# SiftScience/kafka-assigner

Hardware: AMD Instinct MI355X
Metric: assignment scenarios/sec at 100k partitions x 1k brokers RF=3 (higher is better)
Workload: dtype int32

## Files before the change

kafka-assigner_amd/csrc/kas_first_fit.h:

```cpp
#pragma once

namespace kas {

#ifndef KAS_P4_U
#define KAS_P4_U 4
#endif
#ifndef KAS_P4_U_WIDE
#define KAS_P4_U_WIDE 1
#endif
template <int W, int NW, int NC = NW>
KAS_DEV void p4_lists_parallel(const LdsView& L, const TopicView& T, int32_t live_count, int32_t wave,
                               int64_t (&st)[8], int32_t& fail_win, int32_t& fail_row, uint64_t* fin = nullptr, uint64_t fin_hi = 0ull) {
  const int lane = kasw::lane();
  uint64_t* prog = (uint64_t*)&L.ctl[KAS_CTL_PROG];
  int32_t oc[NC], total = 0;
#pragma unroll
  for (int w = 0; w < NC; ++w) { oc[w] = L.ctl[KAS_CTL_OC + w]; total += oc[w]; }
  auto orphan_row = [&](int32_t g) -> int32_t {
    int32_t w = 0, base = 0;
#pragma unroll
    for (int k = 0; k < NC - 1; ++k) {
      const bool next = w == k && g >= base + oc[k];
      base += next ? oc[k] : 0;
      w += next ? 1 : 0;
    }
    return g < total ? T.orph[((int64_t)chunk_begin<NC>(T.nt, w) << 6) + (g - base)] : -1;
  };
  auto row_cells = [&](int32_t p) -> MidRaw<W> {
    return mid_load_raw<W>(T.mid, T.ow, p >= 0 ? p : 0, p >= 0, T.m32);
  };
  const int32_t n_win = (total + 63) >> 6;
  const int32_t dw = (lane >= 1 && lane < NW) ? lane : 1;
  const int32_t xw = (wave + NW - dw) % NW;
  const int32_t cap = T.cap, mw = mid_width(T.ow);
  constexpr int U = W >= 4 ? KAS_P4_U_WIDE : KAS_P4_U;
  int32_t p_nxt = orphan_row(64 * wave + lane);
  MidRaw<W> c_nxt = row_cells(p_nxt);
  for (int32_t w = wave; w < n_win; w += NW) {
    const int32_t p = p_nxt;
    int32_t c_cur[W];
    mid_unpack<W>(c_nxt, T.ow, c_cur, T.m32);
    p_nxt = orphan_row(64 * (w + NW) + lane);
    c_nxt = row_cells(p_nxt);
    kasw::repoll();
    if (kasw::ballot(L.ctl[KAS_CTL_FAILWIN] < w) != 0) break;
    int32_t hc = 0, hr[W];
#pragma unroll
    for (int k = 0; k < W; ++k) {
      hr[k] = (p >= 0 && c_cur[k] >= 0) ? (int32_t)lds_rack(L, c_cur[k]) : -1;
      hc += (p >= 0 && c_cur[k] >= 0) ? 1 : 0;
    }
    int32_t need = p >= 0 ? T.rf - hc : 0;
    int32_t j = kasw::shfl(L.ctl[KAS_CTL_HEAD], 0);
    if (lane == 0) prog[wave] = ((uint64_t)(uint32_t)w << 32) | (uint32_t)j;
    KAS_COUNT(st[4]);
    bool stop = false;
    bool placed = false;
    for (;;) {
      uint64_t pend = kasw::ballot(need > 0);
      if (pend == 0) break;
      if (j >= live_count) {
        if (lane == 0) kasw::lds_atomic_min(&L.ctl[KAS_CTL_FAILWIN], w);
        stop = true;
        break;
      }
      int32_t n[U], slots[U], rk[U];
#pragma unroll
      for (int u = 0; u < U; ++u) n[u] = (int32_t)L.live[j + u < live_count ? j + u : j];
#pragma unroll
      for (int u = 0; u < U; ++u) rk[u] = (int32_t)lds_rack(L, n[u]);
      if (w > 0 && NW > 1) {
        const int32_t upto = j + U < live_count ? j + U : live_count;
        const bool watch = lane >= 1 && lane < NW && w - dw >= 0;
        const uint64_t want = ((uint64_t)(uint32_t)(w - dw) << 32) + (uint32_t)upto;
        bool abandoned = false;
        int32_t idle = 0;
        for (;;) {
          kasw::repoll();
          if (kasw::ballot(watch && prog[xw] < want) == 0) break;
          if (kasw::ballot(L.ctl[KAS_CTL_FAILWIN] < w) != 0) { abandoned = true; break; }
          if (watchdog_poll((uint32_t*)&L.ctl[KAS_CTL_WATCHDOG], false, idle)) {
            if (lane == 0) kasw::lds_atomic_min(&L.ctl[KAS_CTL_FAILWIN], -1);
            abandoned = true;
            break;
          }
        }
        if (abandoned) { stop = true; break; }
      }
#pragma unroll
      for (int u = 0; u < U; ++u) slots[u] = cap - lds_load(L, n[u]);
      int32_t taken[U];
#pragma unroll
      for (int u = 0; u < U; ++u) {
        taken[u] = 0;
        if (j + u < live_count && pend != 0) {
          KAS_COUNT(st[5]);
          if (slots[u] > 0) {
            bool want = need > 0;
#pragma unroll
            for (int k = 0; k < W; ++k) want = want && !(k < hc && hr[k] == rk[u]);
            const uint64_t wm = kasw::ballot(want);
            if (wm != 0) {
              const int32_t rank = kasw::count_below(wm);
              if (want && rank < slots[u]) {
                if (W == 3 && T.m32) {
                  put<W>(c_cur, hc, n[u]);
                  placed = true;
                } else {
                  T.mid[(int64_t)p * mw + hc] = (uint16_t)n[u];
                }
                put<W>(hr, hc, rk[u]);
                hc += 1;
                need -= 1;
              }
              const int32_t takers = kasw::popc(wm);
              taken[u] = takers < slots[u] ? takers : slots[u];
              pend = kasw::ballot(need > 0);
            }
          }
        }
      }
      if (lane == 0) {
#pragma unroll
        for (int u = 0; u < U; ++u) if (taken[u] > 0) lds_load(L, n[u]) = cap - slots[u] + taken[u];
      }
      kasw::lockstep();
      j += U;
      if (lane == 0) prog[wave] = ((uint64_t)(uint32_t)w << 32) | (uint32_t)(j < live_count ? j : live_count);
    }
    if constexpr (W == 3) {
      if (T.m32 && placed) reinterpret_cast<uint32_t*>(T.mid)[p] = mid32_pack(c_cur[0], c_cur[1], c_cur[2]);
    }
    if (stop) {
      if (j >= live_count) {
        const uint64_t left = kasw::ballot(need > 0);
        fail_win = w;
        fail_row = kasw::shfl(p, left != 0 ? kasw::first_lane(left) : 0);
      }
      if (lane == 0) prog[wave] = (uint64_t)(uint32_t)(w + 1) << 32;
      break;
    }
    if (lane == 0) {
      int32_t head = L.ctl[KAS_CTL_HEAD];
      while (head < live_count && lds_load(L, (int32_t)L.live[head]) >= cap) ++head;
      kasw::lds_atomic_max(&L.ctl[KAS_CTL_HEAD], head);
      prog[wave] = (uint64_t)(uint32_t)(w + 1) << 32;
    }
    if (fin != nullptr) {
      const int32_t nxt0 = kasw::shfl(p_nxt, 0);
      kasw::wave_sync();
      if (lane == 0) kasw::store_shared_u64_lds(fin, fin_hi | (uint64_t)(uint32_t)(nxt0 >= 0 ? nxt0 : T.P));
    }
  }
}

KAS_DEV void first_fit_reset_ctl(const LdsView& L, int32_t tid) {
  if (tid < KAS_CTL_INTS) L.ctl[tid] = tid == KAS_CTL_FAILROW ? -1 : (tid == KAS_CTL_FAILWIN ? 0x7fffffff : 0);
}

KAS_DEV int32_t first_fit_live_list(const LdsView& L, const TopicView& T, int32_t idxN) {
  const int lane = kasw::lane();
  const int32_t N = T.N, cap = T.cap;
  const int32_t start = (N - idxN) % N;
  int32_t live_count = 0;
  for (int32_t base = 0; base < N; base += 64) {
    const int32_t j = base + lane;
    int32_t n = j + start; if (n >= N) n -= N;
    const bool is_live = j < N && lds_load(L, n) < cap;
    const uint64_t m = kasw::ballot(is_live);
    if (is_live) L.live[live_count + kasw::count_below(m)] = (int16_t)n;
    live_count += kasw::popc(m);
  }
  kasw::lockstep();
  if (lane == 0) L.ctl[KAS_CTL_LIVE] = live_count;
  return live_count;
}

KAS_DEV bool first_fit_hung(const LdsView& L) { return KAS_SPIN_BOUND > 0 && L.ctl[KAS_CTL_WATCHDOG] != 0; }

KAS_DEV TopicOutcome first_fit_outcome(const LdsView& L, const TopicView& T, bool hung) {
  TopicOutcome o;
  o.status = KAS_OK; o.fail_partition = -1; o.moved_replicas = 0; o.moved_partitions = 0;
  const int32_t row = hung ? -1 : L.ctl[KAS_CTL_FAILROW];
  if (hung) o.status = KAS_FAIL_WATCHDOG;
  else if (row >= 0) {
    o.status = KAS_FAIL_UNASSIGNABLE;
    o.fail_partition = T.pid_arr ? T.pid_arr[row] : row;
  }
  return o;
}

template <int W, int NW, int NC = NW, bool FS = false>
KAS_DEV void first_fit_windows(const LdsView& L, const TopicView& T, int32_t wave, int64_t (&st)[8], uint64_t* fin = nullptr, uint64_t fin_hi = 0ull) {
  const int lane = kasw::lane();
  if constexpr (FS) {
    int32_t total_o = 0;
#pragma unroll
    for (int w = 0; w < NC; ++w) total_o += L.ctl[KAS_CTL_OC + w];
    int32_t first = T.P;
    if (total_o > 0) {
      int32_t w0 = 0;
      while (w0 < NC - 1 && L.ctl[KAS_CTL_OC + w0] == 0) ++w0;
      first = T.orph[(int64_t)chunk_begin<NC>(T.nt, w0) << 6];
    }
    if (lane == 0) kasw::store_shared_u64_lds(fin, fin_hi | (uint64_t)(uint32_t)first);
  }
  int32_t fail_win = -1, fail_row = -1;
  p4_lists_parallel<W, NW, NC>(L, T, L.ctl[KAS_CTL_LIVE], wave, st, fail_win, fail_row, fin, fin_hi);
  if constexpr (FS) kasw::wave_sync(); else kasw::sync();
  if (fail_win >= 0 && fail_win == L.ctl[KAS_CTL_FAILWIN] && lane == 0) L.ctl[KAS_CTL_FAILROW] = fail_row;
}

template <int W, int NW, int NC = NW, bool FS = false>
KAS_DEV TopicOutcome first_fit_topic(const LdsView& L, const TopicView& T, int64_t (&st)[8], uint64_t* fin = nullptr, uint64_t fin_hi = 0ull) {
  static_assert(!FS || NW == 1, "first fit inside the order kernel's workgroup is one wavefront");
  const int32_t wave = FS ? 0 : kasw::wave_id();
  auto barrier = [&]() { if constexpr (FS) kasw::wave_sync(); else kasw::sync(); };
  if (wave == 0) first_fit_live_list(L, T, java_abs_mod(T.hash, T.N));
  barrier();
  first_fit_windows<W, NW, NC, FS>(L, T, wave, st, fin, fin_hi);
  barrier();
  return first_fit_outcome(L, T, first_fit_hung(L));
}

template <int W, int PW, bool FS = false, int M32C = -1>
KAS_DEV void p4_scenario(const KasLaunch& a, int32_t s, unsigned char* lds_raw, uint64_t* fs = nullptr) {
  constexpr int NW = PW, NT = 64 * NW, NC = KAS_P4_WAVES;
  const int lane = kasw::lane();
  const int tid = FS ? lane : kasw::tid();
  auto barrier = [&]() { if constexpr (FS) kasw::wave_sync(); else kasw::sync(); };
  const kas_scenario_desc sd = a.scen[s];
  const int32_t N = sd.n_nodes;
  const KasP4Lds lay = kas_p4_lds_layout(a.n_max);
  LdsView L;
  L.x = nullptr; L.qrs = nullptr; L.idmap = nullptr; L.ids = nullptr; L.ring_p = nullptr; L.ring_meta = nullptr; L.ring_rack = nullptr;
  L.load = (int32_t*)(lds_raw + lay.off_load);
  L.rack = (int16_t*)(lds_raw + lay.off_rack);
  L.live = (int16_t*)(lds_raw + lay.off_live);
  L.ctl = (int32_t*)(lds_raw + lay.off_ctl);
  L.ns = 1; L.rs = 1;
  const int32_t* g_node_rack = a.node_rack + sd.node_off;
  const int64_t t_begin = kasw::clock_ticks();
  int64_t st[8] = {0, 0, 0, 0, 0, 0, 0, 0};
  int32_t* orph = a.orph + a.orph_off[s];
  bool failed = false;
  int32_t moved_r = 0, moved_p = 0;
  for (int32_t k = 0; k < sd.topic_count; ++k) {
    const int32_t ti = sd.topic_begin + k;
    const kas_topic_desc td = a.topics[ti];
    int32_t* const orph_topic = orph;
    orph += (int64_t)((td.n_partitions > 0 ? td.n_partitions : 0) + 63) / 64 * 64;
    if (failed) {
      out_pad(topic_out(a, td), (int64_t)td.n_partitions * td.out_width, tid, NT);
      TopicOutcome o;
      o.status = KAS_SKIPPED; o.fail_partition = -1; o.moved_replicas = 0; o.moved_partitions = 0;
      if (tid == 0) put_topic_result(a, ti, o);
      continue;
    }
    const kas_topic_result tr0 = a.topic_results[ti];
    moved_r += tr0.moved_replicas; moved_p += tr0.moved_partitions;
    const int32_t* p4s = a.p4s + (int64_t)ti * (KAS_P4S_HEAD + a.n_max);
    if (tr0.status != KAS_OK || p4s[0] == 0) {
      if constexpr (FS) {
        if (lane == 0) kasw::store_shared_u64_lds(&fs[0], ((uint64_t)(uint32_t)k << 32) | (uint64_t)(uint32_t)(td.n_partitions > 0 ? td.n_partitions : 0));
      }
      continue;
    }
    TopicView T = topic_view(a, td, N, M32C);
    T.orph = orph_topic;
    T.cap = p4s[1];
    barrier();
    for (int32_t i = tid; i < N; i += NT) { L.load[i] = p4s[KAS_P4S_HEAD + i]; L.rack[i] = (int16_t)g_node_rack[i]; }
    first_fit_reset_ctl(L, tid);
    barrier();
    if (tid < NC) L.ctl[KAS_CTL_OC + tid] = p4s[2 + tid];
    TopicOutcome o = first_fit_topic<W, NW, NC, FS>(L, T, st, FS ? &fs[0] : nullptr, (uint64_t)(uint32_t)k << 32);
    if (o.status != KAS_OK) {
      failed = true;
      moved_r -= tr0.moved_replicas; moved_p -= tr0.moved_partitions;
      if constexpr (FS) {
        if (lane == 0) kasw::store_shared_u64_lds(&fs[1], (uint64_t)(uint32_t)k);
        int32_t idle = 0;
        for (;;) {
          kasw::repoll();
          if (kasw::ballot(kasw::load_shared_u64_lds(&fs[2]) != 0ull) != 0ull) break;
          if (watchdog_poll(reinterpret_cast<uint32_t*>(&fs[3]), false, idle)) break;
        }
      }
      out_pad(topic_out(a, td), (int64_t)td.n_partitions * td.out_width, tid, NT);
      if (tid == 0) {
        put_topic_result(a, ti, o);
        put_scenario_result(a, s, o.status, k, o.fail_partition, moved_r, moved_p);
      }
    }
  }
  if constexpr (FS) {
    kasw::wave_sync();
    if (lane == 0) kasw::store_shared_u64_lds(&fs[0], (uint64_t)(uint32_t)sd.topic_count << 32);
  }
  if (tid == 0 && a.stats) a.stats[(int64_t)s * KAS_STATS_PER_SCENARIO + 3] += kasw::clock_ticks() - t_begin;
}

}
```

Before: 678,000.

## Prefetch orphan lists two windows ahead with async inline-asm global loads

Replaces the per-row orphan-index search with precomputed prefix/step offsets, and issues orphan-list and mid-row loads as asynchronous inline-asm global loads two windows ahead. Waiting is deferred until after the placement loop, so memory latency overlaps with the first-fit work. The new path is used only for single-wave forms with a compile-time M32C. It adds hand-written asm with s_nop and explicit waits, plus template specialisations for full-width rows.

```diff
diff --git a/kafka-assigner_amd/csrc/kas_first_fit.h b/kafka-assigner_amd/csrc/kas_first_fit.h
--- a/kafka-assigner_amd/csrc/kas_first_fit.h
+++ b/kafka-assigner_amd/csrc/kas_first_fit.h
@@ -8,42 +8,123 @@
 #ifndef KAS_P4_U_WIDE
 #define KAS_P4_U_WIDE 1
 #endif
-template <int W, int NW, int NC = NW>
+KAS_DEV void first_fit_request_u32(uint32_t& dst, const void* base, uint32_t voff) {
+#if defined(__HIP_DEVICE_COMPILE__)
+  asm volatile("s_nop 4\n\tglobal_load_dword %0, %1, %2 offset:0" : "+v"(dst) : "v"(voff), "s"(base) : "memory");
+#else
+  kasw::gload_u32_async<0>(dst, base, voff);
+#endif
+}
+KAS_DEV void first_fit_request_u16(uint32_t& dst, const void* base, uint32_t voff) {
+#if defined(__HIP_DEVICE_COMPILE__)
+  asm volatile("s_nop 4\n\tglobal_load_ushort %0, %1, %2 offset:0" : "+v"(dst) : "v"(voff), "s"(base) : "memory");
+#else
+  kasw::gload_u16_async<0>(dst, base, voff);
+#endif
+}
+template <int W, bool M32, bool FULLW>
+KAS_DEV void first_fit_rows_request(MidRaw<W>& r, const uint16_t* mid, int32_t ow, int32_t p) {
+  if constexpr (M32) {
+    first_fit_request_u32(r.w[0], mid, (uint32_t)p * 4u);
+  } else if constexpr (FULLW) {
+    const uint32_t off = (uint32_t)p * (uint32_t)(2 * mid_width_of<W>());
+#pragma unroll
+    for (int k = 0; k < W / 2; ++k) first_fit_request_u32(r.w[k], mid, off + 4u * (uint32_t)k);
+    if constexpr (W & 1) first_fit_request_u16(r.w[W / 2], mid, off + 2u * (uint32_t)(W - 1));
+  } else {
+    const uint32_t off = (uint32_t)p * (uint32_t)(2 * mid_width(ow));
+#pragma unroll
+    for (int k = 0; k < W; ++k) first_fit_request_u16(r.w[k], mid, off + 2u * (uint32_t)(k < ow ? k : ow - 1));
+  }
+}
+template <int W, bool M32, bool FULLW>
+KAS_DEV MidRaw<W> first_fit_rows_take(const MidRaw<W>& r, int32_t ow, bool active) {
+  MidRaw<W> o;
+#pragma unroll
+  for (int k = 0; k < W; ++k) o.w[k] = 0xffffffffu;
+  if constexpr (M32) {
+    if (active) o.w[0] = r.w[0];
+  } else if constexpr (FULLW) {
+#pragma unroll
+    for (int k = 0; k < W / 2; ++k) if (active) o.w[k] = r.w[k];
+    if constexpr (W & 1) if (active) o.w[W / 2] = r.w[W / 2] | 0xffff0000u;
+  } else {
+#pragma unroll
+    for (int k = 0; k < W; ++k) if (active && k < ow) o.w[k] = r.w[k];
+  }
+  return o;
+}
+
+template <int W, int NW, int NC = NW, int AS = -1, bool FULLW = false>
 KAS_DEV void p4_lists_parallel(const LdsView& L, const TopicView& T, int32_t live_count, int32_t wave,
                                int64_t (&st)[8], int32_t& fail_win, int32_t& fail_row, uint64_t* fin = nullptr, uint64_t fin_hi = 0ull) {
+  static_assert(AS < 0 || NW == 1, "the asynchronous requests are the one-wavefront forms'");
+  static_assert(AS != 1 || W == 3, "dword mid rows: lists 3 wide");
   const int lane = kasw::lane();
   uint64_t* prog = (uint64_t*)&L.ctl[KAS_CTL_PROG];
-  int32_t oc[NC], total = 0;
-#pragma unroll
-  for (int w = 0; w < NC; ++w) { oc[w] = L.ctl[KAS_CTL_OC + w]; total += oc[w]; }
-  auto orphan_row = [&](int32_t g) -> int32_t {
-    int32_t w = 0, base = 0;
-#pragma unroll
-    for (int k = 0; k < NC - 1; ++k) {
-      const bool next = w == k && g >= base + oc[k];
-      base += next ? oc[k] : 0;
-      w += next ? 1 : 0;
-    }
-    return g < total ? T.orph[((int64_t)chunk_begin<NC>(T.nt, w) << 6) + (g - base)] : -1;
-  };
-  auto row_cells = [&](int32_t p) -> MidRaw<W> {
-    return mid_load_raw<W>(T.mid, T.ow, p >= 0 ? p : 0, p >= 0, T.m32);
-  };
+  int32_t pre[NC], step[NC], total = 0;
+#pragma unroll
+  for (int k = 0; k < NC; ++k) {
+    pre[k] = total;
+    step[k] = (chunk_begin<NC>(T.nt, k) << 6) - (k > 0 ? (chunk_begin<NC>(T.nt, k - 1) << 6) + kasw::uniform(L.ctl[KAS_CTL_OC + k - 1]) : 0);
+    total += kasw::uniform(L.ctl[KAS_CTL_OC + k]);
+  }
   const int32_t n_win = (total + 63) >> 6;
+  if (wave >= n_win) return;
+  auto orphan_entry = [&](int32_t g) -> uint32_t {
+    int32_t e = g + step[0];
+#pragma unroll
+    for (int k = 1; k < NC; ++k) e += g >= pre[k] ? step[k] : 0;
+    return g < total ? (uint32_t)e : 0u;
+  };
+  const int32_t* const uorph = kasw::uniform_ptr(T.orph);
+  const uint16_t* const umid = kasw::uniform_ptr(T.mid);
+  auto list_request = [&](uint32_t& l, int32_t g) {
+    const uint32_t e = orphan_entry(g);
+    if constexpr (AS >= 0) first_fit_request_u32(l, uorph, e * 4u);
+    else l = (uint32_t)T.orph[e];
+  };
+  auto list_take = [&](uint32_t l, int32_t g) -> int32_t { return g < total ? (int32_t)l : -1; };
+  auto rows_request = [&](MidRaw<W>& r, int32_t p) {
+    if constexpr (AS >= 0) first_fit_rows_request<W, AS == 1, FULLW>(r, umid, T.ow, p >= 0 ? p : 0);
+    else r = mid_load_raw<W>(T.mid, T.ow, p >= 0 ? p : 0, p >= 0, T.m32);
+  };
+  auto rows_take = [&](const MidRaw<W>& r, int32_t p) -> MidRaw<W> {
+    if constexpr (AS >= 0) return first_fit_rows_take<W, AS == 1, FULLW>(r, T.ow, p >= 0);
+    else return r;
+  };
+  auto loads_wait = [&](uint32_t& l, MidRaw<W>& r) {
+    if constexpr (AS >= 0) {
+      kasw::wait_loads();
+      kasw::arrived(l);
+#pragma unroll
+      for (int k = 0; k < W; ++k) kasw::arrived(r.w[k]);
+    }
+  };
   const int32_t dw = (lane >= 1 && lane < NW) ? lane : 1;
   const int32_t xw = (wave + NW - dw) % NW;
   const int32_t cap = T.cap, mw = mid_width(T.ow);
   constexpr int U = W >= 4 ? KAS_P4_U_WIDE : KAS_P4_U;
-  int32_t p_nxt = orphan_row(64 * wave + lane);
-  MidRaw<W> c_nxt = row_cells(p_nxt);
+  uint32_t l_nxt = 0u, l_far = 0u;
+  MidRaw<W> c_nxt;
+#pragma unroll
+  for (int k = 0; k < W; ++k) c_nxt.w[k] = 0xffffffffu;
+  list_request(l_nxt, 64 * wave + lane);
+  list_request(l_far, 64 * (wave + NW) + lane);
+  loads_wait(l_nxt, c_nxt);
+  kasw::arrived(l_far);
+  int32_t p_cur = list_take(l_nxt, 64 * wave + lane);
+  int32_t p_nxt = list_take(l_far, 64 * (wave + NW) + lane);
+  rows_request(c_nxt, p_cur);
+  loads_wait(l_far, c_nxt);
   for (int32_t w = wave; w < n_win; w += NW) {
-    const int32_t p = p_nxt;
+    const int32_t p = p_cur;
     int32_t c_cur[W];
-    mid_unpack<W>(c_nxt, T.ow, c_cur, T.m32);
-    p_nxt = orphan_row(64 * (w + NW) + lane);
-    c_nxt = row_cells(p_nxt);
+    mid_unpack<W>(rows_take(c_nxt, p), T.ow, c_cur, T.m32);
     kasw::repoll();
     if (kasw::ballot(L.ctl[KAS_CTL_FAILWIN] < w) != 0) break;
+    list_request(l_far, 64 * (w + 2 * NW) + lane);
+    rows_request(c_nxt, p_nxt);
     int32_t hc = 0, hr[W];
 #pragma unroll
     for (int k = 0; k < W; ++k) {
@@ -128,6 +209,7 @@
       j += U;
       if (lane == 0) prog[wave] = ((uint64_t)(uint32_t)w << 32) | (uint32_t)(j < live_count ? j : live_count);
     }
+    loads_wait(l_far, c_nxt);
     if constexpr (W == 3) {
       if (T.m32 && placed) reinterpret_cast<uint32_t*>(T.mid)[p] = mid32_pack(c_cur[0], c_cur[1], c_cur[2]);
     }
@@ -151,6 +233,8 @@
       kasw::wave_sync();
       if (lane == 0) kasw::store_shared_u64_lds(fin, fin_hi | (uint64_t)(uint32_t)(nxt0 >= 0 ? nxt0 : T.P));
     }
+    p_cur = p_nxt;
+    p_nxt = list_take(l_far, 64 * (w + 2 * NW) + lane);
   }
 }
 
@@ -190,7 +274,7 @@
   return o;
 }
 
-template <int W, int NW, int NC = NW, bool FS = false>
+template <int W, int NW, int NC = NW, bool FS = false, int AS = -1>
 KAS_DEV void first_fit_windows(const LdsView& L, const TopicView& T, int32_t wave, int64_t (&st)[8], uint64_t* fin = nullptr, uint64_t fin_hi = 0ull) {
   const int lane = kasw::lane();
   if constexpr (FS) {
@@ -206,19 +290,24 @@
     if (lane == 0) kasw::store_shared_u64_lds(fin, fin_hi | (uint64_t)(uint32_t)first);
   }
   int32_t fail_win = -1, fail_row = -1;
-  p4_lists_parallel<W, NW, NC>(L, T, L.ctl[KAS_CTL_LIVE], wave, st, fail_win, fail_row, fin, fin_hi);
+  if constexpr (AS == 0) {
+    if (T.ow == W) p4_lists_parallel<W, NW, NC, 0, true>(L, T, L.ctl[KAS_CTL_LIVE], wave, st, fail_win, fail_row, fin, fin_hi);
+    else p4_lists_parallel<W, NW, NC, 0, false>(L, T, L.ctl[KAS_CTL_LIVE], wave, st, fail_win, fail_row, fin, fin_hi);
+  } else {
+    p4_lists_parallel<W, NW, NC, AS>(L, T, L.ctl[KAS_CTL_LIVE], wave, st, fail_win, fail_row, fin, fin_hi);
+  }
   if constexpr (FS) kasw::wave_sync(); else kasw::sync();
   if (fail_win >= 0 && fail_win == L.ctl[KAS_CTL_FAILWIN] && lane == 0) L.ctl[KAS_CTL_FAILROW] = fail_row;
 }
 
-template <int W, int NW, int NC = NW, bool FS = false>
+template <int W, int NW, int NC = NW, bool FS = false, int AS = -1>
 KAS_DEV TopicOutcome first_fit_topic(const LdsView& L, const TopicView& T, int64_t (&st)[8], uint64_t* fin = nullptr, uint64_t fin_hi = 0ull) {
   static_assert(!FS || NW == 1, "first fit inside the order kernel's workgroup is one wavefront");
   const int32_t wave = FS ? 0 : kasw::wave_id();
   auto barrier = [&]() { if constexpr (FS) kasw::wave_sync(); else kasw::sync(); };
   if (wave == 0) first_fit_live_list(L, T, java_abs_mod(T.hash, T.N));
   barrier();
-  first_fit_windows<W, NW, NC, FS>(L, T, wave, st, fin, fin_hi);
+  first_fit_windows<W, NW, NC, FS, AS>(L, T, wave, st, fin, fin_hi);
   barrier();
   return first_fit_outcome(L, T, first_fit_hung(L));
 }
@@ -274,7 +363,7 @@
     first_fit_reset_ctl(L, tid);
     barrier();
     if (tid < NC) L.ctl[KAS_CTL_OC + tid] = p4s[2 + tid];
-    TopicOutcome o = first_fit_topic<W, NW, NC, FS>(L, T, st, FS ? &fs[0] : nullptr, (uint64_t)(uint32_t)k << 32);
+    TopicOutcome o = first_fit_topic<W, NW, NC, FS, (NW == 1 && M32C >= 0) ? M32C : -1>(L, T, st, FS ? &fs[0] : nullptr, (uint64_t)(uint32_t)k << 32);
     if (o.status != KAS_OK) {
       failed = true;
       moved_r -= tr0.moved_replicas; moved_p -= tr0.moved_partitions;
```

Result: faster. 699,300, median of 6 (+3.1%).
